# 0xPolygonZero/plonky2

Measured on NVIDIA H100. Metric: goldilocks_field_elements_per_s_ntt_lde_merkle, higher is better.
Workload: dtype u64

## Files before the change

include/plonky2_b200.h:

```cpp
#ifndef PLONKY2_B200_H
#define PLONKY2_B200_H
#include <stddef.h>
#include <stdint.h>

#ifdef __cplusplus
extern "C" {
#endif

#define GL_OK 0
#define GL_ERR_BAD_SHAPE 1
#define GL_ERR_OOM 2
#define GL_ERR_CUDA 3
#define GL_ERR_UNSUPPORTED 4
#define GL_ERR_BAD_ARG 5
#define GL_ERR_POW_FAILED 6
#define GL_ERR_DIV_ZERO 7

#define GL_MEM_HOST 0
#define GL_MEM_DEVICE 1

#define GL_SALT_SIZE 4

typedef struct gl_ctx gl_ctx;
typedef struct gl_commit gl_commit;
typedef struct gl_merkle gl_merkle;
typedef struct gl_fri gl_fri;

int gl_ctx_create(int device, void* stream, gl_ctx** out);
void gl_ctx_destroy(gl_ctx* ctx);
const char* gl_last_error(const gl_ctx* ctx);
int gl_ctx_synchronize(gl_ctx* ctx);
int gl_ctx_device_bytes(gl_ctx* ctx, uint64_t* in_use, uint64_t* high, int reset_high);
void* gl_ctx_stream(const gl_ctx* ctx);
uint64_t gl_ctx_launch_count(const gl_ctx* ctx);
int gl_ctx_set_ntt_group(gl_ctx* ctx, uint32_t columns);
#define GL_PHASE_INTT 0
#define GL_PHASE_LDE 1
#define GL_PHASE_LEAF_HASH 2
#define GL_PHASE_MERKLE_LEVELS 3
#define GL_NUM_PHASES 4
int gl_ctx_set_profiling(gl_ctx* ctx, int on);
int gl_ctx_phase_ms(gl_ctx* ctx, int phase, double* ms, uint64_t* count);
int gl_ctx_reset_phases(gl_ctx* ctx);

int gl_ntt(gl_ctx* ctx, uint64_t* data, uint32_t log_n, uint32_t batch, size_t stride, int inverse,
           uint32_t zero_factor_log, uint64_t coset_shift, int mem);

int gl_ntt_bcast(gl_ctx* ctx, const uint64_t* in, size_t in_stride, uint32_t log_n, uint32_t batch, int inverse,
                 uint64_t* const* outs, uint32_t n_outs, size_t out_stride);

int gl_bcast(gl_ctx* ctx, const uint64_t* src, size_t words, uint64_t* const* dests, uint32_t n_dests, uint32_t max_ctas);

int gl_commit_create(gl_ctx* ctx, const uint64_t* cols, size_t col_stride, uint32_t B, uint32_t log_n,
                     uint32_t rate_bits, uint32_t cap_height, const uint64_t* salt, int is_coeffs,
                     int mem, gl_commit** out);
int gl_commit_create_sharded(gl_ctx* ctx, const uint64_t* cols, size_t col_stride, uint32_t B, uint32_t log_n,
                             uint32_t rate_bits, uint32_t cap_height, const uint64_t* salt, int is_coeffs,
                             int mem, uint32_t shard_index, uint32_t num_shards, gl_commit** out);
#define GL_COLS_VALUES 0
#define GL_COLS_COEFFS 1
#define GL_COLS_COEFFS_CANONICAL 2
int gl_commit_begin(gl_ctx* ctx, uint32_t B, uint32_t log_n, uint32_t rate_bits, uint32_t cap_height, int blinding,
                    uint32_t shard_index, uint32_t num_shards, uint64_t* coeff_storage, gl_commit** out);
int gl_commit_add_columns(gl_commit* c, uint32_t first_col, uint32_t count, const uint64_t* cols, size_t col_stride,
                          int kind, int mem);
int gl_commit_finish(gl_commit* c, const uint64_t* salt, int mem);
int gl_commit_finish_keyed(gl_commit* c, const uint8_t key[32]);
int gl_commit_finish_prefixed(gl_commit* c, const uint64_t* prefix);
int gl_commit_begin_blocked(gl_ctx* ctx, uint32_t B, uint32_t log_n, uint32_t rate_bits, uint32_t cap_height,
                            uint32_t num_blocks, uint64_t* coeff_storage, gl_commit** out);
uint32_t gl_commit_lde_blocks(const gl_commit* c);
int gl_commit_shard(const gl_commit* c, uint32_t* shard_index, uint32_t* num_shards);
void gl_commit_destroy(gl_commit* c);
uint32_t gl_commit_num_polys(const gl_commit* c);
uint32_t gl_commit_leaf_width(const gl_commit* c);
uint32_t gl_commit_degree_log(const gl_commit* c);
uint32_t gl_commit_rate_bits(const gl_commit* c);
uint32_t gl_commit_cap_height(const gl_commit* c);
int gl_commit_cap(gl_commit* c, uint64_t* out, int mem);
int gl_commit_coeffs(gl_commit* c, uint64_t* out, int mem);
int gl_commit_leaves(gl_commit* c, size_t row_begin, size_t row_count, uint64_t* out, int mem);
int gl_commit_digests(gl_commit* c, uint64_t* out, int mem);
int gl_commit_get_lde_values(gl_commit* c, size_t index, size_t step, uint64_t* out);
int gl_commit_open(gl_commit* c, const uint64_t* leaf_indices, size_t count, uint64_t* out_leaves,
                   uint64_t* out_paths);
int gl_commit_eval_ext(gl_commit* c, const uint64_t point[2], uint64_t* out);
int gl_openings(gl_ctx* ctx, gl_commit* const* commits, const uint32_t* point_index, size_t n_evals,
                const uint64_t* points, size_t n_points, uint64_t* out, int mem);
int gl_openings_shard(gl_ctx* ctx, gl_commit* const* commits, const uint32_t* point_index, size_t n_evals,
                      const uint64_t* points, size_t n_points, uint32_t shard_index, uint32_t num_shards, uint64_t* out,
                      int mem);
const uint64_t* gl_commit_dev_lde(const gl_commit* c, size_t* col_stride);
const uint64_t* gl_commit_dev_coeffs(const gl_commit* c);
// ... 143 lines not shown
```

plonky2_b200/_native.py:

```python
import ctypes as C
import os

import numpy as np

HERE = os.path.dirname(os.path.abspath(__file__))
LIB_PATH = os.path.join(HERE, "libplonky2_b200.so")

GL_OK = 0
GL_ERR_BAD_SHAPE, GL_ERR_OOM, GL_ERR_CUDA, GL_ERR_UNSUPPORTED, GL_ERR_BAD_ARG, GL_ERR_POW_FAILED, GL_ERR_DIV_ZERO = 1, 2, 3, 4, 5, 6, 7
MEM_HOST, MEM_DEVICE = 0, 1
COLS_VALUES, COLS_COEFFS, COLS_COEFFS_CANONICAL = 0, 1, 2

u64p = C.POINTER(C.c_uint64)
u32p = C.POINTER(C.c_uint32)
vp = C.c_void_p

EXPORTS = [
    "gl_ctx_create", "gl_ctx_destroy", "gl_last_error", "gl_ctx_synchronize", "gl_ctx_launch_count",
    "gl_ctx_set_ntt_group", "gl_ctx_set_profiling", "gl_ctx_phase_ms", "gl_ctx_reset_phases", "gl_ctx_stream", "gl_ntt",
    "gl_ntt_bcast", "gl_bcast", "gl_commit_create", "gl_commit_create_sharded", "gl_commit_begin", "gl_commit_add_columns",
    "gl_commit_finish", "gl_commit_shard", "gl_commit_destroy", "gl_commit_num_polys",
    "gl_commit_leaf_width", "gl_commit_degree_log", "gl_commit_rate_bits", "gl_commit_cap_height",
    "gl_commit_cap", "gl_commit_coeffs", "gl_commit_leaves", "gl_commit_digests", "gl_commit_get_lde_values",
    "gl_commit_open", "gl_commit_eval_ext", "gl_openings", "gl_openings_shard", "gl_stark_quotient", "gl_stark_quotient_aux", "gl_stark_quotient_shard", "gl_stark_quotient_from_shards", "gl_stark_lookup_helpers", "gl_stark_ctl_helpers", "gl_plonk_quotient", "gl_plonk_quotient_shard", "gl_lookup_polys", "gl_sigma_polys", "gl_commit_dev_lde", "gl_commit_dev_coeffs", "gl_partial_products_and_zs", "gl_poseidon_permute_host",
    "gl_poseidon_permute_many", "gl_poseidon_hash_many", "gl_poseidon_hash_no_pad_many", "gl_poseidon_two_to_one_many", "gl_merkle_build", "gl_merkle_destroy",
    "gl_merkle_cap", "gl_merkle_digests", "gl_merkle_open", "gl_fri_begin", "gl_fri_begin_values", "gl_fri_values_local", "gl_fri_begin_from_coeffs",
    "gl_fri_destroy", "gl_fri_coeffs", "gl_fri_commit_round", "gl_fri_commit_round_sharded", "gl_fri_mix", "gl_fri_fold", "gl_fri_final_poly",
    "gl_fri_open", "gl_fri_num_rounds", "gl_fri_pow", "gl_commit_finish_keyed", "gl_random_field_elements",
    "gl_commit_finish_prefixed", "gl_commit_dev_cap", "gl_commit_begin_blocked", "gl_commit_lde_blocks",
    "gl_ctx_device_bytes",
]


class FriBatch(C.Structure):
    _fields_ = [("point", C.c_uint64 * 2), ("num_polys", C.c_size_t), ("oracle_index", u32p),
                ("poly_index", u32p)]


class ShapeError(ValueError):
    """Mirrors the reference's shape panics (fft.rs:171-177, merkle_tree.rs:195-200, oracle.rs:128)."""


class NativeError(RuntimeError):
    pass


_lib = None


def lib():
    global _lib
    if _lib is not None:
        return _lib
    if not os.path.exists(LIB_PATH):
        raise NativeError(
            "libplonky2_b200.so is not built (run `python -c 'import __graft_entry__ as g; g.build()'`); "
            "plonky2_b200 has no CPU fallback")
    L = C.CDLL(LIB_PATH)
    L.gl_ctx_create.argtypes = [C.c_int, vp, C.POINTER(vp)]
    L.gl_ctx_destroy.argtypes = [vp]
    L.gl_ctx_destroy.restype = None
    L.gl_last_error.argtypes = [vp]
    L.gl_last_error.restype = C.c_char_p
    L.gl_ctx_synchronize.argtypes = [vp]
    L.gl_ctx_device_bytes.argtypes = [vp, u64p, u64p, C.c_int]
    L.gl_ctx_launch_count.argtypes = [vp]
    L.gl_ctx_launch_count.restype = C.c_uint64
    L.gl_ctx_set_ntt_group.argtypes = [vp, C.c_uint32]
    L.gl_ntt.argtypes = [vp, vp, C.c_uint32, C.c_uint32, C.c_size_t, C.c_int, C.c_uint32, C.c_uint64, C.c_int]
    L.gl_ctx_stream.argtypes = [vp]
    L.gl_ctx_stream.restype = vp
    L.gl_ntt_bcast.argtypes = [vp, vp, C.c_size_t, C.c_uint32, C.c_uint32, C.c_int, C.POINTER(vp), C.c_uint32, C.c_size_t]
    L.gl_bcast.argtypes = [vp, vp, C.c_size_t, C.POINTER(vp), C.c_uint32, C.c_uint32]
    L.gl_commit_begin.argtypes = [vp, C.c_uint32, C.c_uint32, C.c_uint32, C.c_uint32, C.c_int, C.c_uint32, C.c_uint32,
                                  vp, C.POINTER(vp)]
    L.gl_commit_begin_blocked.argtypes = [vp, C.c_uint32, C.c_uint32, C.c_uint32, C.c_uint32, C.c_uint32, vp,
                                          C.POINTER(vp)]
    L.gl_commit_add_columns.argtypes = [vp, C.c_uint32, C.c_uint32, vp, C.c_size_t, C.c_int, C.c_int]
    L.gl_commit_finish.argtypes = [vp, vp, C.c_int]
    L.gl_commit_finish_keyed.argtypes = [vp, C.c_char_p]
    L.gl_commit_finish_prefixed.argtypes = [vp, vp]
    L.gl_random_field_elements.argtypes = [vp, C.c_char_p, C.c_uint32, C.c_uint64, C.c_size_t, vp, C.c_int]
    L.gl_commit_create.argtypes = [vp, vp, C.c_size_t, C.c_uint32, C.c_uint32, C.c_uint32, C.c_uint32, vp,
                                   C.c_int, C.c_int, C.POINTER(vp)]
    L.gl_commit_create_sharded.argtypes = [vp, vp, C.c_size_t, C.c_uint32, C.c_uint32, C.c_uint32, C.c_uint32, vp,
                                           C.c_int, C.c_int, C.c_uint32, C.c_uint32, C.POINTER(vp)]
    L.gl_commit_shard.argtypes = [vp, u32p, u32p]
    L.gl_ctx_set_profiling.argtypes = [vp, C.c_int]
    L.gl_ctx_phase_ms.argtypes = [vp, C.c_int, C.POINTER(C.c_double), C.POINTER(C.c_uint64)]
    L.gl_ctx_reset_phases.argtypes = [vp]
    L.gl_commit_destroy.argtypes = [vp]
    L.gl_commit_destroy.restype = None
    for n in ("gl_commit_num_polys", "gl_commit_leaf_width", "gl_commit_degree_log", "gl_commit_rate_bits",
              "gl_commit_cap_height", "gl_commit_lde_blocks"):
        getattr(L, n).argtypes = [vp]
        getattr(L, n).restype = C.c_uint32
    L.gl_commit_cap.argtypes = [vp, vp, C.c_int]
    L.gl_commit_coeffs.argtypes = [vp, vp, C.c_int]
    L.gl_commit_leaves.argtypes = [vp, C.c_size_t, C.c_size_t, vp, C.c_int]
    L.gl_commit_digests.argtypes = [vp, vp, C.c_int]
    L.gl_commit_get_lde_values.argtypes = [vp, C.c_size_t, C.c_size_t, vp]
    L.gl_commit_open.argtypes = [vp, vp, C.c_size_t, vp, vp]
    L.gl_commit_eval_ext.argtypes = [vp, vp, vp]
    L.gl_openings.argtypes = [vp, C.POINTER(vp), u32p, C.c_size_t, vp, C.c_size_t, vp, C.c_int]
    L.gl_openings_shard.argtypes = [vp, C.POINTER(vp), u32p, C.c_size_t, vp, C.c_size_t, C.c_uint32, C.c_uint32, vp,
                                    C.c_int]
    L.gl_stark_quotient.argtypes = [vp, vp, vp, C.c_uint32, vp, C.c_uint32, vp, C.c_uint32, C.c_uint32, vp]
    L.gl_stark_quotient_aux.argtypes = [vp, vp, vp, vp, C.c_uint32, vp, C.c_uint32, vp, C.c_uint32, C.c_uint32, vp]
    L.gl_stark_quotient_shard.argtypes = [vp, vp, vp, vp, C.c_uint32, vp, C.c_uint32, vp, C.c_uint32, C.c_uint32, vp]
    L.gl_stark_quotient_from_shards.argtypes = [vp, vp, C.c_uint32, C.c_uint32, C.c_uint32, C.c_uint32, vp]
    L.gl_stark_lookup_helpers.argtypes = [vp, vp, C.c_size_t, C.c_uint32, C.c_uint32, vp, u32p, C.c_uint32, vp,
                                          C.c_uint32, vp, C.c_uint32, C.c_uint32, vp]
    L.gl_stark_ctl_helpers.argtypes = [vp, vp, C.c_size_t, C.c_uint32, C.c_uint32, vp, u32p, C.c_uint32, vp, C.c_uint32,
                                       vp, C.c_uint32, C.c_uint32, u32p, vp]
    L.gl_plonk_quotient.argtypes = [vp, vp, C.c_uint32, vp, C.c_uint32, vp, C.c_uint32, vp, C.c_uint32, C.c_uint32,
                                    C.c_uint32, vp]
    L.gl_plonk_quotient_shard.argtypes = [vp, vp, C.c_uint32, vp, C.c_uint32, vp, C.c_uint32, vp, C.c_uint32,
                                          C.c_uint32, C.c_uint32, vp]
    L.gl_lookup_polys.argtypes = [vp, vp, C.c_uint32, C.c_uint32, C.c_uint32, vp, u32p, C.c_uint32, vp, C.c_int]
    L.gl_sigma_polys.argtypes = [vp, vp, C.c_size_t, C.c_int, C.c_uint32, C.c_uint32, C.c_uint32, C.c_uint64, vp, vp,
                                 C.c_int]
# ... 60 lines not shown

class Handle:
    destroyer = None
    h = None

    def close(self):
        if self.h:
            getattr(lib(), self.destroyer)(self.h)
            self.h = None

    def __del__(self):
        try:
            self.close()
        except Exception:
            pass


class Context(Handle):
    destroyer = "gl_ctx_destroy"
    _torch_stream = None

    def __init__(self, device=0, stream=None):
        h = vp()
        check(lib().gl_ctx_create(int(device), vp(stream) if stream else None, C.byref(h)))
        self.h = h
        self.device = device

    def synchronize(self):
        check(lib().gl_ctx_synchronize(self.h), self.h)

    def after_caller(self):
        import torch

        if self._torch_stream is None:
            self._torch_stream = torch.cuda.ExternalStream(self.stream, device=torch.device("cuda", self.device))
        self._torch_stream.wait_stream(torch.cuda.current_stream(self._torch_stream.device))

    @property
    def stream(self):
        return int(lib().gl_ctx_stream(self.h) or 0)

    def device_bytes(self, reset_high=False):
        in_use, high = C.c_uint64(), C.c_uint64()
        check(lib().gl_ctx_device_bytes(self.h, C.byref(in_use), C.byref(high), int(bool(reset_high))), self.h)
        return in_use.value, high.value

    @property
    def launch_count(self):
        return int(lib().gl_ctx_launch_count(self.h))

    def set_ntt_group(self, columns):
        check(lib().gl_ctx_set_ntt_group(self.h, int(columns)), self.h)

    PHASES = {"intt": 0, "lde": 1, "leaf_hash": 2, "merkle_levels": 3}

    def set_profiling(self, on):
        check(lib().gl_ctx_set_profiling(self.h, int(bool(on))), self.h)

    def reset_phases(self):
        check(lib().gl_ctx_reset_phases(self.h), self.h)

    def phase_ms(self):
        out = {}
        for name, pid in self.PHASES.items():
            ms, cnt = C.c_double(), C.c_uint64()
            check(lib().gl_ctx_phase_ms(self.h, pid, C.byref(ms), C.byref(cnt)), self.h)
            out[name] = (ms.value, cnt.value)
        return out


_default_ctx = {}


def default_context(device=0):
    if device not in _default_ctx:
        _default_ctx[device] = Context(device)
    return _default_ctx[device]
```

plonky2_b200/csrc/plonky2_b200.cu:

```cuda
#include <cooperative_groups.h>
#include <cub/device/device_radix_sort.cuh>
#include <cuda_runtime.h>

#include <cstdarg>
#include <cstdio>
#include <cstring>
#include <functional>
#include <initializer_list>
#include <map>
#include <memory>
#include <set>
#include <string>
#include <tuple>
#include <vector>

#include <sys/random.h>

#include <cerrno>

#include "../../include/plonky2_b200.h"
#include "gl_chacha.cuh"
#include "gl_field.cuh"
#include "gl_logup.cuh"
#include "gl_ctl.cuh"
#include "gl_ntt.cuh"
#include "gl_poseidon.cuh"
#include "gl_sigma.cuh"
#include "gl_vanishing.cuh"

using namespace gl;
typedef uint64_t u64;

static thread_local std::string g_last_error;

struct gl_ctx {
    int device = 0;
    cudaStream_t stream = nullptr;
    bool own_stream = false;
    u64 launches = 0;
    std::string err;
    std::map<std::tuple<int, u64, u64>, u64*> step_tabs;
    std::map<std::tuple<int, int, u64>, u64*> post_tabs;
    size_t table_bytes = 0;
    std::map<int, u64*> fold_tabs;
    cudaStream_t copy_stream = nullptr;
    std::set<const void*> smem_attr_done;
    u64* scratch = nullptr;
    size_t scratch_words = 0;
    u64* pinned = nullptr;
    size_t pinned_words = 0;
    u64* dstage = nullptr;
    size_t dstage_words = 0;
    uint32_t ntt_group = 0;
    int ntt_variant = 0;
    bool lde_per_coset = false;
    int sm_count = 0;
    int coop_ok = 0;
    int coop_blocks_per_sm = 0;
    bool prof_on = false;
    struct Pending {
        int phase;
        cudaEvent_t a, b;
    };
    std::vector<Pending> prof_pending;
    double prof_ms[GL_NUM_PHASES] = {0};
    u64 prof_count[GL_NUM_PHASES] = {0};
};

struct PhaseScope {
    gl_ctx* ctx;
    cudaEvent_t a = nullptr, b = nullptr;
    int phase;
    PhaseScope(gl_ctx* c, int ph) : ctx(c), phase(ph) {
        if (!ctx->prof_on) return;
        cudaEventCreate(&a);
        cudaEventCreate(&b);
        cudaEventRecord(a, ctx->stream);
    }
    ~PhaseScope() {
        if (!a) return;
        cudaEventRecord(b, ctx->stream);
        ctx->prof_pending.push_back({phase, a, b});
    }
};

static int set_err(gl_ctx* ctx, int code, const char* fmt, ...) {
    char buf[512];
    va_list ap;
    va_start(ap, fmt);
    vsnprintf(buf, sizeof(buf), fmt, ap);
    va_end(ap);
    g_last_error = buf;
    if (ctx) ctx->err = buf;
    return code;
}
#define CK(ctx, call)                                                                          \
    do {                                                                                       \
        cudaError_t e_ = (call);                                                               \
// ... 334 lines not shown
    }
}
__global__ void k_tree_open_prefixed(TreeView t, const u64* prefix, const u64* indices, u64* out_leaves,
                                     u64* out_paths) {
    const size_t idx = indices[blockIdx.x];
    const uint32_t num_layers = t.log_n - t.cap_height;
    const uint32_t lw = t.W + 4;
    for (uint32_t k = threadIdx.x; k < lw; k += blockDim.x)
        out_leaves[(size_t)blockIdx.x * lw + k] =
            canon(k < 4 ? prefix[4 * idx + k] : t.leaves[idx * t.ls + (size_t)(k - 4) * t.es]);
    const size_t L = (size_t)1 << num_layers;
    const size_t tree_index = idx >> num_layers;
    const u64* sub = t.digests + 4 * (tree_index * 2 * (L - 1));
    for (uint32_t k = threadIdx.x; k < num_layers * 4; k += blockDim.x) {
        const uint32_t i = k >> 2, w = k & 3;
        const size_t node = (idx & (L - 1)) >> i;
        out_paths[(size_t)blockIdx.x * num_layers * 4 + k] = sub[4 * digest_pos(node ^ 1, i) + w];
    }
}

struct Tree {
    u64* leaves = nullptr;
    u64* base = nullptr;
    bool own_leaves = false;
    u64* digests = nullptr;
    u64* cap = nullptr;
    u64* prefix = nullptr;
    size_t N = 0;
    size_t ls = 0, es = 1;
    uint32_t W = 0, log_n = 0, cap_height = 0;
    TreeView view() const { return TreeView{leaves, digests, cap, N, ls ? ls : (size_t)W, es, W, log_n, cap_height}; }
    size_t digest_words() const { return 8 * (N - ((size_t)1 << cap_height)); }
    size_t cap_words() const { return (size_t)4 << cap_height; }
};

static int log2_exact(size_t n, uint32_t* out) {
    if (n == 0 || (n & (n - 1))) return 1;
    uint32_t l = 0;
    while (((size_t)1 << l) < n) l++;
    *out = l;
    return 0;
}

static int tree_hash(gl_ctx* ctx, const Tree& t);
static int tree_build(gl_ctx* ctx, Tree& t) {
    if (log2_exact(t.N, &t.log_n)) return set_err(ctx, GL_ERR_BAD_SHAPE, "Not a power of two: %zu", t.N);
    if (t.cap_height > t.log_n)
        return set_err(ctx, GL_ERR_BAD_SHAPE, "cap_height=%u should be at most log2(leaves.len())=%u", t.cap_height,
                       t.log_n);
    TRY(dmalloc(ctx, &t.digests, t.digest_words()));
    TRY(dmalloc(ctx, &t.cap, t.cap_words()));
    return tree_hash(ctx, t);
}
static int tree_hash(gl_ctx* ctx, const Tree& t) {
    TreeView v = t.view();
    {
        PhaseScope ps(ctx, GL_PHASE_LEAF_HASH);
        const int cta = HASH_CTA;
        if (t.prefix)
            k_leaf_hash_prefixed<<<(unsigned)((t.N + cta - 1) / cta), cta, 0, ctx->stream>>>(v, t.prefix);
        else
            k_leaf_hash<<<(unsigned)((t.N + cta - 1) / cta), cta, 0, ctx->stream>>>(v);
        CKL(ctx);
    }
    PhaseScope ps2(ctx, GL_PHASE_MERKLE_LEVELS);
    const uint32_t sub_log = t.log_n - t.cap_height;
    const size_t coop_threads = ctx->coop_ok ? (size_t)ctx->coop_blocks_per_sm * ctx->sm_count * HASH_CTA : 0;
    for (uint32_t i = 1; i <= sub_log; i++) {
        size_t total = (size_t)1 << (t.log_n - i);
        if (coop_threads && total <= coop_threads && i < sub_log) {
            unsigned nb = (unsigned)((total + HASH_CTA - 1) / HASH_CTA);
            uint32_t i0 = i;
            void* args[] = {(void*)&v, (void*)&i0};
            CK(ctx, cudaLaunchCooperativeKernel((void*)k_merkle_upper, dim3(nb), dim3(HASH_CTA), args, 0, ctx->stream));
            ctx->launches++;
            break;
        }
        const int cta = HASH_CTA;
        k_merkle_level<<<(unsigned)((total + cta - 1) / cta), cta, 0, ctx->stream>>>(v, i);
        CKL(ctx);
    }
    return GL_OK;
}
static void tree_free(gl_ctx* ctx, Tree& t) {
    if (t.own_leaves) dfree(ctx, t.base ? t.base : t.leaves);
    dfree(ctx, t.digests);
    dfree(ctx, t.cap);
    dfree(ctx, t.prefix);
    t.leaves = t.digests = t.cap = t.prefix = nullptr;
}
static int tree_open(gl_ctx* ctx, const Tree& t, const u64* leaf_indices, size_t count, u64* out_leaves,
                     u64* out_paths) {
    if (count == 0) return GL_OK;
    for (size_t i = 0; i < count; i++)
        if (leaf_indices[i] >= t.N) return set_err(ctx, GL_ERR_BAD_ARG, "leaf index %llu out of range",
                                                   (unsigned long long)leaf_indices[i]);
    const uint32_t layers = t.log_n - t.cap_height;
    const size_t lw = count * (t.W + (t.prefix ? 4 : 0)), pw = count * layers * 4;
    TRY(ensure_dstage(ctx, count + lw + pw));
    TRY(ensure_pinned(ctx, count + lw + pw));
    CK(ctx, cudaStreamSynchronize(ctx->stream));
    memcpy(ctx->pinned, leaf_indices, count * 8);
    TRY(h2d(ctx, ctx->dstage, ctx->pinned, count));
    if (t.prefix)
        k_tree_open_prefixed<<<(unsigned)count, 128, 0, ctx->stream>>>(t.view(), t.prefix, ctx->dstage,
                                                                      ctx->dstage + count, ctx->dstage + count + lw);
    else
        k_tree_open<<<(unsigned)count, 128, 0, ctx->stream>>>(t.view(), ctx->dstage, ctx->dstage + count,
                                                             ctx->dstage + count + lw);
    CKL(ctx);
    TRY(d2h(ctx, ctx->pinned, ctx->dstage + count, lw + pw));
    memcpy(out_leaves, ctx->pinned, lw * 8);
    if (pw) memcpy(out_paths, ctx->pinned + lw, pw * 8);
    return GL_OK;
}

struct gl_commit {
    gl_ctx* ctx;
    uint32_t B, W, degree_log, rate_bits;
    uint32_t shard_index = 0, shard_log = 0;
    uint32_t lde_blocks = 0, block_log = 0;
    bool blinding;
    u64* coeffs = nullptr;
    bool own_coeffs = true;
    bool finished = false;
    Tree tree;
};

__global__ void k_salt(const u64* salt, size_t N, uint32_t log_N, size_t row0, size_t rows, u64* lde, size_t lde_stride,
                       uint32_t B) {
    size_t j = (size_t)blockIdx.x * blockDim.x + threadIdx.x;
    if (j >= rows) return;
    size_t i = (size_t)(__brevll(row0 + j) >> (64 - log_N));
    if (log_N == 0) i = 0;
    for (int s = 0; s < GL_SALT_SIZE; s++) lde[(size_t)(B + s) * lde_stride + j] = canon(salt[(size_t)s * N + i]);
}
__global__ void k_rows_from_columns(const u64* lde, size_t lde_stride, size_t row0, size_t rows, uint32_t W, u64* out) {
    __shared__ u64 tile[32][33];
    const size_t rb = (size_t)blockIdx.x * 32;
    const uint32_t kb = blockIdx.y * 32;
    for (int i = threadIdx.y; i < 32; i += blockDim.y) {
        const size_t r = rb + threadIdx.x;
        const uint32_t k = kb + i;
        if (r < rows && k < W) tile[i][threadIdx.x] = lde[(size_t)k * lde_stride + row0 + r];
    }
    __syncthreads();
    for (int i = threadIdx.y; i < 32; i += blockDim.y) {
        const size_t r = rb + i;
        const uint32_t k = kb + threadIdx.x;
        if (r < rows && k < W) out[r * W + k] = tile[threadIdx.x][i];
    }
}
__global__ void k_fold_coeffs(const u64* coeffs, size_t stride, size_t n, size_t M, u64 sM, u64* out) {
    size_t k0 = (size_t)blockIdx.x * blockDim.x + threadIdx.x;
    if (k0 >= M) return;
    const u64* col = coeffs + (size_t)blockIdx.y * stride;
    u64 acc = 0;
    for (size_t k1 = n / M; k1-- > 0;) acc = mul_add(acc, sM, col[k0 + M * k1]);
    out[(size_t)blockIdx.y * M + k0] = acc;
}
__global__ void k_canon(u64* data, size_t n) {
    size_t i = (size_t)blockIdx.x * blockDim.x + threadIdx.x;
    if (i < n) data[i] = canon(data[i]);
}
static int coset_lde_columns(gl_ctx* ctx, const u64* coeffs, uint32_t ncols, uint32_t log_n, uint32_t log_M, u64 shift,
                             u64* out, size_t out_stride) {
    const size_t n = (size_t)1 << log_n;
    if (log_M >= log_n) return lde_columns(ctx, coeffs, n, ncols, (int)log_n, (int)(log_M - log_n), shift, out, out_stride);
    const size_t M = (size_t)1 << log_M;
    DevBuf folded(ctx);
    TRY(folded.alloc((size_t)ncols * M));
    for (uint32_t b0 = 0; b0 < ncols; b0 += MAX_GRID_Y) {
        const uint32_t bc = (ncols - b0 < MAX_GRID_Y) ? ncols - b0 : MAX_GRID_Y;
        k_fold_coeffs<<<dim3((unsigned)((M + 127) / 128), bc), 128, 0, ctx->stream>>>(
            coeffs + (size_t)b0 * n, n, n, M, gl::pow(shift, M), folded.get() + (size_t)b0 * M);
        CKL(ctx);
    }
    return lde_columns(ctx, folded.get(), M, ncols, (int)log_M, 0, shift, out, out_stride);
}

static int commit_alloc(gl_ctx* ctx, gl_commit* c, uint32_t cap_height, u64* ext_coeffs) {
    const size_t n = (size_t)1 << c->degree_log, N = n << c->rate_bits;
    if (ext_coeffs) {
        c->coeffs = ext_coeffs;
        c->own_coeffs = false;
    } else {
        TRY(dmalloc(ctx, &c->coeffs, (size_t)c->B * n));
    }
    const uint32_t sl = c->shard_log;
    const size_t Nloc = N >> sl;
    Tree& t = c->tree;
    t.N = Nloc;
    t.W = c->W;
    t.log_n = c->degree_log + c->rate_bits - sl;
    t.cap_height = cap_height - sl;
    t.ls = 1;
    t.es = Nloc;
    if (c->lde_blocks) return GL_OK;
    t.own_leaves = true;
    TRY(dmalloc(ctx, &t.leaves, Nloc * (size_t)c->W));
    return GL_OK;
}
static int commit_extend(gl_ctx* ctx, const gl_commit* c, uint32_t g0, uint32_t gc, uint32_t g, uint32_t s, u64* out,
                         size_t out_stride) {
    PhaseScope ps(ctx, GL_PHASE_LDE);
    const u64 shift =
        mul(MULTIPLICATIVE_GROUP_GENERATOR, gl::pow(root_of_unity(c->degree_log + c->rate_bits), bitrev32(g, s)));
    return coset_lde_columns(ctx, c->coeffs + ((size_t)g0 << c->degree_log), gc, c->degree_log,
                             c->degree_log + c->rate_bits - s, shift, out, out_stride);
}
static int commit_chunk(gl_ctx* ctx, gl_commit* c, uint32_t g0, uint32_t gc, int kind) {
    const size_t n = (size_t)1 << c->degree_log;
    Tree& t = c->tree;
    u64* cg = c->coeffs + (size_t)g0 * n;
    if (kind == 0) {
        PhaseScope ps(ctx, GL_PHASE_INTT);
        TRY(ntt_natural(ctx, cg, n, cg, n, (int)c->degree_log, gc, true, 1));
    } else if (kind == 1) {
        size_t tot = (size_t)gc * n;
        k_canon<<<(unsigned)((tot + 255) / 256), 256, 0, ctx->stream>>>(cg, tot);
        CKL(ctx);
    }
    if (c->lde_blocks) return GL_OK;
    return commit_extend(ctx, c, g0, gc, c->shard_index, c->shard_log, t.leaves + (size_t)g0 * t.N, t.N);
}
static int commit_block(gl_ctx* ctx, const gl_commit* c, uint32_t g, DevBuf& scratch, Tree* out) {
    Tree t = c->tree;
    t.N >>= c->block_log;
    t.log_n -= c->block_log;
    t.cap_height -= c->block_log;
    t.es = t.N;
    if (t.cap) {
        t.digests += (size_t)g * t.digest_words();
        t.cap += (size_t)g * t.cap_words();
    }
    if (c->lde_blocks) {
        if (!scratch.get()) TRY(scratch.alloc((size_t)c->W * t.N));
        TRY(commit_extend(ctx, c, 0, c->B, g, c->block_log, scratch.get(), t.N));
        t.leaves = scratch.get();
    }
    *out = t;
    return GL_OK;
}
static int commit_finish(gl_ctx* ctx, gl_commit* c, const u64* salt, int mem, const ChaChaKey* key) {
    Tree& t = c->tree;
    const size_t Nloc = t.N;
    const uint32_t log_N = c->degree_log + c->rate_bits;
    HostReads reads(ctx);
    if (salt) {
        DevBuf dsalt(ctx);
        u64* sp;
        TRY(device_in(ctx, salt, (size_t)GL_SALT_SIZE << log_N, mem, dsalt, &sp));
        TRY(reads.mark(ctx->stream, mem));
        k_salt<<<(unsigned)((Nloc + 255) / 256), 256, 0, ctx->stream>>>(sp, (size_t)1 << log_N, log_N,
                                                                       (size_t)c->shard_index * Nloc, Nloc, t.leaves,
                                                                       Nloc, c->B);
        CKL(ctx);
    } else if (key) {
        const size_t items = salt_fill_items(log_N, Nloc);
        k_chacha_salt<<<dim3((unsigned)((items + 255) / 256), GL_SALT_SIZE), 256, 0, ctx->stream>>>(
            *key, log_N, (u64)c->shard_index * Nloc, Nloc, t.leaves + (size_t)c->B * Nloc, Nloc);
        CKL(ctx);
    }
    TRY(dmalloc(ctx, &t.digests, t.digest_words()));
    TRY(dmalloc(ctx, &t.cap, t.cap_words()));
    DevBuf scratch(ctx);
    for (uint32_t g = 0; g < (1u << c->block_log); g++) {
        Tree b;
        TRY(commit_block(ctx, c, g, scratch, &b));
        TRY(tree_hash(ctx, b));
    }
    TRY(reads.wait());
    c->finished = true;
    return GL_OK;
}
static int os_random_key(gl_ctx* ctx, uint8_t out[32]) {
    size_t got = 0;
    while (got < 32) {
        const ssize_t r = getrandom(out + got, 32 - got, 0);
        if (r < 0) {
            if (errno == EINTR) continue;
            return set_err(ctx, GL_ERR_UNSUPPORTED, "getrandom failed: %s", strerror(errno));
        }
        got += (size_t)r;
    }
    return GL_OK;
}

struct PolyRef {
    const u64* ptr;
    u64 a0, a1;
};
__global__ void k_fri_compose(const PolyRef* refs, uint32_t num, size_t n, u64* comp ) {
    size_t k = (size_t)blockIdx.x * blockDim.x + threadIdx.x;
    if (k >= n) return;
    Acc160 a0 = {0, 0, 0}, a1 = {0, 0, 0};
    for (uint32_t j = 0; j < num; j++) {
        const u64 c = refs[j].ptr[k];
        acc_mul(a0, c, refs[j].a0);
        acc_mul(a1, c, refs[j].a1);
    }
    comp[2 * k] = acc_reduce(a0);
    comp[2 * k + 1] = acc_reduce(a1);
}
__device__ __forceinline__ E2 e2_pow_tab(const u64* hi, const u64* lo, size_t m) {
    const size_t h = m >> 12, l = m & 4095;
    return e2_mul(E2{hi[2 * h], hi[2 * h + 1]}, E2{lo[2 * l], lo[2 * l + 1]});
}
__global__ void k_fill_e2_pows(E2 base, size_t count, u64* out) {
    size_t i = (size_t)blockIdx.x * blockDim.x + threadIdx.x;
    if (i >= count) return;
    E2 r = e2_pow(base, i);
    out[2 * i] = r.a;
    out[2 * i + 1] = r.b;
}
struct E2Pows4 {
    E2 base[4];
    size_t count[4];
    u64* out[4];
};
__global__ void k_fill_e2_pows4(E2Pows4 p) {
    size_t i = (size_t)blockIdx.x * blockDim.x + threadIdx.x;
#pragma unroll
// ... 729 lines not shown

extern "C" {

int gl_ctx_create(int device, void* stream, gl_ctx** out) {
    if (!out) return set_err(nullptr, GL_ERR_BAD_ARG, "out is NULL");
    *out = nullptr;
    int count = 0;
    cudaError_t e = cudaGetDeviceCount(&count);
    if (e != cudaSuccess || count == 0)
        return set_err(nullptr, GL_ERR_CUDA, "no CUDA device available (%s); this library has no CPU fallback",
                       cudaGetErrorString(e));
    if (device < 0 || device >= count) return set_err(nullptr, GL_ERR_BAD_ARG, "device %d out of range", device);
    gl_ctx* ctx = new gl_ctx();
    ctx->device = device;
    auto init = [&]() -> int {
        CK(ctx, cudaSetDevice(device));
        if (stream) {
            ctx->stream = (cudaStream_t)stream;
        } else {
            CK(ctx, cudaStreamCreateWithFlags(&ctx->stream, cudaStreamNonBlocking));
            ctx->own_stream = true;
        }
        CK(ctx, cudaDeviceGetAttribute(&ctx->sm_count, cudaDevAttrMultiProcessorCount, device));
        CK(ctx, cudaDeviceGetAttribute(&ctx->coop_ok, cudaDevAttrCooperativeLaunch, device));
        if (cudaOccupancyMaxActiveBlocksPerMultiprocessor(&ctx->coop_blocks_per_sm, k_merkle_upper, HASH_CTA, 0) !=
            cudaSuccess)
            ctx->coop_blocks_per_sm = 0;
        const PoseidonTables& t = host_poseidon_tables();
        CK(ctx, cudaMemcpyToSymbol(c_pos, &t, sizeof(PoseidonTables)));
        return GL_OK;
    };
    const int rc_init = init();
    if (rc_init != GL_OK) {
        if (ctx->own_stream) cudaStreamDestroy(ctx->stream);
        delete ctx;
        return rc_init;
    }
    cudaMemPool_t pool;
    if (cudaDeviceGetDefaultMemPool(&pool, device) == cudaSuccess) {
        unsigned long long thr = ~0ULL;
        cudaMemPoolSetAttribute(pool, cudaMemPoolAttrReleaseThreshold, &thr);
    }
    *out = ctx;
    return GL_OK;
}
void gl_ctx_destroy(gl_ctx* ctx) {
    if (!ctx) return;
    cudaSetDevice(ctx->device);
    cudaStreamSynchronize(ctx->stream);
    for (auto& kv : ctx->step_tabs) cudaFreeAsync(kv.second, ctx->stream);
    for (auto& kv : ctx->post_tabs) cudaFreeAsync(kv.second, ctx->stream);
    for (auto& kv : ctx->fold_tabs) cudaFreeAsync(kv.second, ctx->stream);
    if (ctx->copy_stream) cudaStreamDestroy(ctx->copy_stream);
    if (ctx->scratch) cudaFreeAsync(ctx->scratch, ctx->stream);
    if (ctx->dstage) cudaFreeAsync(ctx->dstage, ctx->stream);
    if (ctx->pinned) cudaFreeHost(ctx->pinned);
    cudaStreamSynchronize(ctx->stream);
    if (ctx->own_stream) cudaStreamDestroy(ctx->stream);
    delete ctx;
}
const char* gl_last_error(const gl_ctx* ctx) { return ctx ? ctx->err.c_str() : g_last_error.c_str(); }
int gl_ctx_synchronize(gl_ctx* ctx) {
    CK(ctx, cudaStreamSynchronize(ctx->stream));
    return GL_OK;
}
int gl_ctx_device_bytes(gl_ctx* ctx, uint64_t* in_use, uint64_t* high, int reset_high) {
    if (!ctx) return set_err(ctx, GL_ERR_BAD_ARG, "null context");
    CK(ctx, cudaSetDevice(ctx->device));
    CK(ctx, cudaStreamSynchronize(ctx->stream));
    cudaMemPool_t pool;
    CK(ctx, cudaDeviceGetDefaultMemPool(&pool, ctx->device));
    uint64_t v = 0;
    CK(ctx, cudaMemPoolGetAttribute(pool, cudaMemPoolAttrUsedMemCurrent, &v));
    if (in_use) *in_use = v;
    CK(ctx, cudaMemPoolGetAttribute(pool, cudaMemPoolAttrUsedMemHigh, &v));
    if (high) *high = v;
    if (reset_high) {
        uint64_t zero = 0;
        CK(ctx, cudaMemPoolSetAttribute(pool, cudaMemPoolAttrUsedMemHigh, &zero));
    }
    return GL_OK;
}
uint64_t gl_ctx_launch_count(const gl_ctx* ctx) { return ctx->launches; }
int gl_ctx_set_ntt_group(gl_ctx* ctx, uint32_t columns) {
    ctx->ntt_variant = (columns >> 31) & 1;
    ctx->lde_per_coset = (columns >> 30) & 1;
    ctx->ntt_group = columns & 0x3FFFFFFFu;
    return GL_OK;
}
int gl_ctx_set_profiling(gl_ctx* ctx, int on) {
    ctx->prof_on = on != 0;
    return GL_OK;
}
int gl_ctx_phase_ms(gl_ctx* ctx, int phase, double* ms, uint64_t* count) {
    if (phase < 0 || phase >= GL_NUM_PHASES) return set_err(ctx, GL_ERR_BAD_ARG, "bad phase");
    if (!ctx->prof_pending.empty()) {
        CK(ctx, cudaStreamSynchronize(ctx->stream));
        for (auto& p : ctx->prof_pending) {
            float t = 0;
            cudaEventElapsedTime(&t, p.a, p.b);
            ctx->prof_ms[p.phase] += t;
            ctx->prof_count[p.phase]++;
            cudaEventDestroy(p.a);
            cudaEventDestroy(p.b);
        }
        ctx->prof_pending.clear();
    }
    if (ms) *ms = ctx->prof_ms[phase];
    if (count) *count = ctx->prof_count[phase];
    return GL_OK;
}
int gl_ctx_reset_phases(gl_ctx* ctx) {
    TRY(gl_ctx_phase_ms(ctx, 0, nullptr, nullptr));
    for (int i = 0; i < GL_NUM_PHASES; i++) {
        ctx->prof_ms[i] = 0;
        ctx->prof_count[i] = 0;
    }
    return GL_OK;
}

int gl_ntt(gl_ctx* ctx, uint64_t* data, uint32_t log_n, uint32_t batch, size_t stride, int inverse,
           uint32_t zero_factor_log, uint64_t coset_shift, int mem) {
    (void)zero_factor_log;
    if (!ctx || !data) return set_err(ctx, GL_ERR_BAD_ARG, "null argument");
    CK(ctx, cudaSetDevice(ctx->device));
    if (log_n > 3 * NTT_MAX_LOG_PASS) return set_err(ctx, GL_ERR_UNSUPPORTED, "log_n %u > 30", log_n);
    const size_t n = (size_t)1 << log_n;
    if (batch > 1 && stride < n) return set_err(ctx, GL_ERR_BAD_SHAPE, "stride %zu < n %zu", stride, n);
    if (canon(coset_shift) == 0) return set_err(ctx, GL_ERR_BAD_ARG, "coset_shift must be non-zero");
    if (mem == GL_MEM_DEVICE) return ntt_natural(ctx, data, stride, data, stride, (int)log_n, batch, inverse != 0, coset_shift);
    DevBuf d(ctx);
    TRY(d.alloc((size_t)batch * n));
    const size_t pitch = (batch > 1 ? stride : n) * 8;
    if (cudaMemcpy2DAsync(d.get(), n * 8, data, pitch, n * 8, batch, cudaMemcpyHostToDevice, ctx->stream) != cudaSuccess)
        return set_err(ctx, GL_ERR_CUDA, "H2D: %s", cudaGetErrorString(cudaGetLastError()));
    TRY(ntt_natural(ctx, d.get(), n, d.get(), n, (int)log_n, batch, inverse != 0, coset_shift));
    cudaError_t e = cudaMemcpy2DAsync(data, pitch, d.get(), n * 8, n * 8, batch, cudaMemcpyDeviceToHost, ctx->stream);
    if (e != cudaSuccess) return set_err(ctx, GL_ERR_CUDA, "D2H: %s", cudaGetErrorString(e));
    if (cudaStreamSynchronize(ctx->stream) != cudaSuccess)
        return set_err(ctx, GL_ERR_CUDA, "sync failed: %s", cudaGetErrorString(cudaGetLastError()));
    return GL_OK;
// ... 79 lines not shown
                    uint32_t shard_index, uint32_t num_shards, uint64_t* coeff_storage, gl_commit** out) {
    if (!ctx || !out) return set_err(ctx, GL_ERR_BAD_ARG, "null argument");
    *out = nullptr;
    uint32_t shard_log = 0;
    TRY(commit_check_shape(ctx, B, log_n, rate_bits, cap_height, shard_index, num_shards, &shard_log));
    CK(ctx, cudaSetDevice(ctx->device));
    CommitPtr c = commit_new(ctx, B, log_n, rate_bits, blinding != 0, shard_index, shard_log);
    TRY(commit_alloc(ctx, c.get(), cap_height, coeff_storage));
    *out = c.release();
    return GL_OK;
}
int gl_commit_begin_blocked(gl_ctx* ctx, uint32_t B, uint32_t log_n, uint32_t rate_bits, uint32_t cap_height,
                            uint32_t num_blocks, uint64_t* coeff_storage, gl_commit** out) {
    if (!ctx || !out) return set_err(ctx, GL_ERR_BAD_ARG, "null argument");
    *out = nullptr;
    uint32_t shard_log = 0, block_log = 0;
    TRY(commit_check_shape(ctx, B, log_n, rate_bits, cap_height, 0, 1, &shard_log));
    if (log2_exact(num_blocks, &block_log) || block_log > cap_height)
        return set_err(ctx, GL_ERR_BAD_SHAPE,
                       "num_blocks=%u: a power of two of at most the cap size 2^%u (blocks own whole cap subtrees)",
                       num_blocks, cap_height);
    CK(ctx, cudaSetDevice(ctx->device));
    CommitPtr c = commit_new(ctx, B, log_n, rate_bits, false, 0, 0);
    c->lde_blocks = num_blocks;
    c->block_log = block_log;
    TRY(commit_alloc(ctx, c.get(), cap_height, coeff_storage));
    *out = c.release();
    return GL_OK;
}
#define NEED_HANDLE(c)                                                         \
    do {                                                                       \
        if (!(c)) return set_err(nullptr, GL_ERR_BAD_ARG, "null handle");       \
    } while (0)
#define NEED_FINISHED(c)                                                                                     \
    do {                                                                                                     \
        NEED_HANDLE(c);                                                                                      \
        if (!(c)->finished) return set_err((c)->ctx, GL_ERR_BAD_ARG, "gl_commit_finish has not been called"); \
    } while (0)
int gl_commit_add_columns(gl_commit* c, uint32_t first_col, uint32_t count, const uint64_t* cols, size_t col_stride,
                          int kind, int mem) {
    NEED_HANDLE(c);
    gl_ctx* ctx = c->ctx;
    if (c->finished) return set_err(ctx, GL_ERR_BAD_ARG, "commitment already finished");
    if (!cols || kind < 0 || kind > 2) return set_err(ctx, GL_ERR_BAD_ARG, "bad argument");
    if (count == 0) return GL_OK;
    if ((size_t)first_col + count > c->B) return set_err(ctx, GL_ERR_BAD_SHAPE, "columns %u..%u outside the batch of %u", first_col, first_col + count, c->B);
    const size_t n = (size_t)1 << c->degree_log;
    if (count > 1 && col_stride < n) return set_err(ctx, GL_ERR_BAD_SHAPE, "Polynomial degrees inconsistent (stride < n)");
    CK(ctx, cudaSetDevice(ctx->device));
    u64* dst = c->coeffs + (size_t)first_col * n;
    const uint32_t CH = 32, CH0 = 8;
    if (mem != GL_MEM_HOST || count <= CH) {
        HostReads reads(ctx);
        if (!(mem == GL_MEM_DEVICE && cols == dst && (col_stride == n || count == 1)))
            CK(ctx, cudaMemcpy2DAsync(dst, n * 8, cols, col_stride * 8, n * 8, count,
                                      mem == GL_MEM_HOST ? cudaMemcpyHostToDevice : cudaMemcpyDeviceToDevice,
                                      ctx->stream));
        TRY(reads.mark(ctx->stream, mem));
        TRY(commit_chunk(ctx, c, first_col, count, kind));
        return reads.wait();
    }
    struct EventList {
        std::vector<cudaEvent_t> v;
        ~EventList() {
            for (auto e : v) cudaEventDestroy(e);
        }
    } evs;
    std::vector<std::pair<uint32_t, uint32_t>> chunks;
    for (uint32_t k0 = 0; k0 < count;) {
        const uint32_t want = k0 == 0 ? CH0 : CH, kc = (count - k0 < want) ? count - k0 : want;
        chunks.emplace_back(k0, kc);
        k0 += kc;
    }
    if (!ctx->copy_stream) CK(ctx, cudaStreamCreateWithFlags(&ctx->copy_stream, cudaStreamNonBlocking));
    cudaEvent_t ready;
    CK(ctx, cudaEventCreateWithFlags(&ready, cudaEventDisableTiming));
    CK(ctx, cudaEventRecord(ready, ctx->stream));
    CK(ctx, cudaStreamWaitEvent(ctx->copy_stream, ready, 0));
    cudaEventDestroy(ready);
    for (auto& ch : chunks) {
        const uint32_t k0 = ch.first, kc = ch.second;
        if (col_stride == n) {
            CK(ctx, cudaMemcpyAsync(dst + (size_t)k0 * n, cols + (size_t)k0 * n, (size_t)kc * n * 8,
                                    cudaMemcpyHostToDevice, ctx->copy_stream));
        } else {
            CK(ctx, cudaMemcpy2DAsync(dst + (size_t)k0 * n, n * 8, cols + (size_t)k0 * col_stride, col_stride * 8, n * 8,
                                      kc, cudaMemcpyHostToDevice, ctx->copy_stream));
        }
        cudaEvent_t e;
        CK(ctx, cudaEventCreateWithFlags(&e, cudaEventDisableTiming));
        CK(ctx, cudaEventRecord(e, ctx->copy_stream));
        evs.v.push_back(e);
    }
    HostReads reads(ctx);
    TRY(reads.mark(ctx->copy_stream, mem));
    for (size_t k = 0; k < chunks.size(); k++) {
        CK(ctx, cudaStreamWaitEvent(ctx->stream, evs.v[k], 0));
        TRY(commit_chunk(ctx, c, first_col + chunks[k].first, chunks[k].second, kind));
    }
    return reads.wait();
}
int gl_commit_finish(gl_commit* c, const uint64_t* salt, int mem) {
    NEED_HANDLE(c);
    gl_ctx* ctx = c->ctx;
    if (c->finished) return set_err(ctx, GL_ERR_BAD_ARG, "commitment already finished");
    if (c->blinding != (salt != nullptr)) return set_err(ctx, GL_ERR_BAD_ARG, "salt must be given exactly when blinding was requested");
    CK(ctx, cudaSetDevice(ctx->device));
    return commit_finish(ctx, c, salt, mem, nullptr);
}
int gl_commit_finish_prefixed(gl_commit* c, const uint64_t* prefix) {
    NEED_HANDLE(c);
    gl_ctx* ctx = c->ctx;
// ... 1462 lines not shown
```

Before: 8.491 billion.

## Overlap coset LDE with leaf hashing on a side stream; skip device copy before INTT

Adds an optional pipelined commit path that splits the LDE into power-of-two coset blocks. Each block is computed on a separate priority stream while the previous block's leaves are hashed, synchronised with events, and the Merkle levels are then built once. It also lets the inverse NTT read device value columns directly instead of first copying them into the coefficient buffer, which removes one device-to-device copy. The pipeline is controlled by a new commit_blocks setting that defaults to 1, so it stays off unless configured; when on, it adds stream and event overhead and smaller per-block kernels.

```diff
diff --git a/include/plonky2_b200.h b/include/plonky2_b200.h
--- a/include/plonky2_b200.h
+++ b/include/plonky2_b200.h
@@ -34,11 +34,13 @@
 void* gl_ctx_stream(const gl_ctx* ctx);
 uint64_t gl_ctx_launch_count(const gl_ctx* ctx);
 int gl_ctx_set_ntt_group(gl_ctx* ctx, uint32_t columns);
+int gl_ctx_set_commit_blocks(gl_ctx* ctx, uint32_t blocks);
 #define GL_PHASE_INTT 0
 #define GL_PHASE_LDE 1
 #define GL_PHASE_LEAF_HASH 2
 #define GL_PHASE_MERKLE_LEVELS 3
-#define GL_NUM_PHASES 4
+#define GL_PHASE_LDE_UNDER_HASH 4
+#define GL_NUM_PHASES 5
 int gl_ctx_set_profiling(gl_ctx* ctx, int on);
 int gl_ctx_phase_ms(gl_ctx* ctx, int phase, double* ms, uint64_t* count);
 int gl_ctx_reset_phases(gl_ctx* ctx);
diff --git a/plonky2_b200/_native.py b/plonky2_b200/_native.py
--- a/plonky2_b200/_native.py
+++ b/plonky2_b200/_native.py
@@ -28,7 +28,7 @@
     "gl_fri_destroy", "gl_fri_coeffs", "gl_fri_commit_round", "gl_fri_commit_round_sharded", "gl_fri_mix", "gl_fri_fold", "gl_fri_final_poly",
     "gl_fri_open", "gl_fri_num_rounds", "gl_fri_pow", "gl_commit_finish_keyed", "gl_random_field_elements",
     "gl_commit_finish_prefixed", "gl_commit_dev_cap", "gl_commit_begin_blocked", "gl_commit_lde_blocks",
-    "gl_ctx_device_bytes",
+    "gl_ctx_device_bytes", "gl_ctx_set_commit_blocks",
 ]
 
 
@@ -67,6 +67,7 @@
     L.gl_ctx_launch_count.argtypes = [vp]
     L.gl_ctx_launch_count.restype = C.c_uint64
     L.gl_ctx_set_ntt_group.argtypes = [vp, C.c_uint32]
+    L.gl_ctx_set_commit_blocks.argtypes = [vp, C.c_uint32]
     L.gl_ntt.argtypes = [vp, vp, C.c_uint32, C.c_uint32, C.c_size_t, C.c_int, C.c_uint32, C.c_uint64, C.c_int]
     L.gl_ctx_stream.argtypes = [vp]
     L.gl_ctx_stream.restype = vp
@@ -233,6 +234,9 @@
     def set_ntt_group(self, columns):
         check(lib().gl_ctx_set_ntt_group(self.h, int(columns)), self.h)
 
+    def set_commit_blocks(self, blocks):
+        check(lib().gl_ctx_set_commit_blocks(self.h, int(blocks)), self.h)
+
     PHASES = {"intt": 0, "lde": 1, "leaf_hash": 2, "merkle_levels": 3}
 
     def set_profiling(self, on):
diff --git a/plonky2_b200/csrc/plonky2_b200.cu b/plonky2_b200/csrc/plonky2_b200.cu
--- a/plonky2_b200/csrc/plonky2_b200.cu
+++ b/plonky2_b200/csrc/plonky2_b200.cu
@@ -44,6 +44,9 @@
     size_t table_bytes = 0;
     std::map<int, u64*> fold_tabs;
     cudaStream_t copy_stream = nullptr;
+    uint32_t commit_blocks = 1;
+    cudaStream_t lde_stream = nullptr;
+    int lde_stream_priority = 0;
     std::set<const void*> smem_attr_done;
     u64* scratch = nullptr;
     size_t scratch_words = 0;
@@ -484,17 +487,25 @@
     TRY(dmalloc(ctx, &t.cap, t.cap_words()));
     return tree_hash(ctx, t);
 }
+static int leaf_hash(gl_ctx* ctx, const Tree& t) {
+    const int cta = HASH_CTA;
+    if (t.prefix)
+        k_leaf_hash_prefixed<<<(unsigned)((t.N + cta - 1) / cta), cta, 0, ctx->stream>>>(t.view(), t.prefix);
+    else
+        k_leaf_hash<<<(unsigned)((t.N + cta - 1) / cta), cta, 0, ctx->stream>>>(t.view());
+    CKL(ctx);
+    return GL_OK;
+}
+static int merkle_levels(gl_ctx* ctx, const Tree& t);
 static int tree_hash(gl_ctx* ctx, const Tree& t) {
-    TreeView v = t.view();
     {
         PhaseScope ps(ctx, GL_PHASE_LEAF_HASH);
-        const int cta = HASH_CTA;
-        if (t.prefix)
-            k_leaf_hash_prefixed<<<(unsigned)((t.N + cta - 1) / cta), cta, 0, ctx->stream>>>(v, t.prefix);
-        else
-            k_leaf_hash<<<(unsigned)((t.N + cta - 1) / cta), cta, 0, ctx->stream>>>(v);
-        CKL(ctx);
-    }
+        TRY(leaf_hash(ctx, t));
+    }
+    return merkle_levels(ctx, t);
+}
+static int merkle_levels(gl_ctx* ctx, const Tree& t) {
+    TreeView v = t.view();
     PhaseScope ps2(ctx, GL_PHASE_MERKLE_LEVELS);
     const uint32_t sub_log = t.log_n - t.cap_height;
     const size_t coop_threads = ctx->coop_ok ? (size_t)ctx->coop_blocks_per_sm * ctx->sm_count * HASH_CTA : 0;
@@ -513,6 +524,21 @@
         CKL(ctx);
     }
     return GL_OK;
+}
+static Tree block_view(const Tree& t, uint32_t s, uint32_t g) {
+    Tree b = t;
+    b.own_leaves = false;
+    b.N >>= s;
+    b.log_n -= s;
+    b.cap_height -= s;
+    const size_t row0 = (size_t)g * b.N;
+    if (b.leaves) b.leaves += row0 * (b.ls ? b.ls : b.W);
+    if (b.prefix) b.prefix += 4 * row0;
+    if (b.cap) {
+        b.digests += (size_t)g * b.digest_words();
+        b.cap += (size_t)g * b.cap_words();
+    }
+    return b;
 }
 static void tree_free(gl_ctx* ctx, Tree& t) {
     if (t.own_leaves) dfree(ctx, t.base ? t.base : t.leaves);
@@ -552,6 +578,7 @@
     uint32_t B, W, degree_log, rate_bits;
     uint32_t shard_index = 0, shard_log = 0;
     uint32_t lde_blocks = 0, block_log = 0;
+    uint32_t pipe_log = 0;
     bool blinding;
     u64* coeffs = nullptr;
     bool own_coeffs = true;
@@ -611,6 +638,13 @@
     return lde_columns(ctx, folded.get(), M, ncols, (int)log_M, 0, shift, out, out_stride);
 }
 
+static uint32_t pipeline_log(uint32_t blocks, uint32_t rate_bits, uint32_t cap_height) {
+    uint32_t want = 0;
+    while ((2u << want) <= blocks) want++;
+    if (want > rate_bits) want = rate_bits;
+    if (want > cap_height) want = cap_height;
+    return want;
+}
 static int commit_alloc(gl_ctx* ctx, gl_commit* c, uint32_t cap_height, u64* ext_coeffs) {
     const size_t n = (size_t)1 << c->degree_log, N = n << c->rate_bits;
     if (ext_coeffs) {
@@ -629,50 +663,122 @@
     t.ls = 1;
     t.es = Nloc;
     if (c->lde_blocks) return GL_OK;
+    c->pipe_log = pipeline_log(ctx->commit_blocks, c->rate_bits > sl ? c->rate_bits - sl : 0, t.cap_height);
     t.own_leaves = true;
     TRY(dmalloc(ctx, &t.leaves, Nloc * (size_t)c->W));
     return GL_OK;
 }
 static int commit_extend(gl_ctx* ctx, const gl_commit* c, uint32_t g0, uint32_t gc, uint32_t g, uint32_t s, u64* out,
                          size_t out_stride) {
-    PhaseScope ps(ctx, GL_PHASE_LDE);
     const u64 shift =
         mul(MULTIPLICATIVE_GROUP_GENERATOR, gl::pow(root_of_unity(c->degree_log + c->rate_bits), bitrev32(g, s)));
     return coset_lde_columns(ctx, c->coeffs + ((size_t)g0 << c->degree_log), gc, c->degree_log,
                              c->degree_log + c->rate_bits - s, shift, out, out_stride);
 }
-static int commit_chunk(gl_ctx* ctx, gl_commit* c, uint32_t g0, uint32_t gc, int kind) {
+static int commit_chunk(gl_ctx* ctx, gl_commit* c, uint32_t g0, uint32_t gc, int kind, const u64* src = nullptr,
+                        size_t src_stride = 0) {
     const size_t n = (size_t)1 << c->degree_log;
     Tree& t = c->tree;
     u64* cg = c->coeffs + (size_t)g0 * n;
     if (kind == 0) {
         PhaseScope ps(ctx, GL_PHASE_INTT);
-        TRY(ntt_natural(ctx, cg, n, cg, n, (int)c->degree_log, gc, true, 1));
+        TRY(ntt_natural(ctx, src ? src : cg, src ? src_stride : n, cg, n, (int)c->degree_log, gc, true, 1));
     } else if (kind == 1) {
         size_t tot = (size_t)gc * n;
         k_canon<<<(unsigned)((tot + 255) / 256), 256, 0, ctx->stream>>>(cg, tot);
         CKL(ctx);
     }
-    if (c->lde_blocks) return GL_OK;
+    if (c->lde_blocks || c->pipe_log) return GL_OK;
+    PhaseScope ps(ctx, GL_PHASE_LDE);
     return commit_extend(ctx, c, g0, gc, c->shard_index, c->shard_log, t.leaves + (size_t)g0 * t.N, t.N);
 }
 static int commit_block(gl_ctx* ctx, const gl_commit* c, uint32_t g, DevBuf& scratch, Tree* out) {
-    Tree t = c->tree;
-    t.N >>= c->block_log;
-    t.log_n -= c->block_log;
-    t.cap_height -= c->block_log;
-    t.es = t.N;
-    if (t.cap) {
-        t.digests += (size_t)g * t.digest_words();
-        t.cap += (size_t)g * t.cap_words();
-    }
+    Tree t = block_view(c->tree, c->block_log, g);
     if (c->lde_blocks) {
         if (!scratch.get()) TRY(scratch.alloc((size_t)c->W * t.N));
+        PhaseScope ps(ctx, GL_PHASE_LDE);
         TRY(commit_extend(ctx, c, 0, c->B, g, c->block_log, scratch.get(), t.N));
         t.leaves = scratch.get();
+        t.es = t.N;
     }
     *out = t;
     return GL_OK;
+}
+class OnStream {
+  public:
+    OnStream(gl_ctx* ctx, cudaStream_t s) : ctx_(ctx), saved_(ctx->stream) { ctx->stream = s; }
+    OnStream(const OnStream&) = delete;
+    OnStream& operator=(const OnStream&) = delete;
+    ~OnStream() { ctx_->stream = saved_; }
+
+  private:
+    gl_ctx* ctx_;
+    cudaStream_t saved_;
+};
+class SideEvents {
+  public:
+    SideEvents(gl_ctx* ctx, cudaStream_t side) : ctx_(ctx), side_(side) {}
+    SideEvents(const SideEvents&) = delete;
+    SideEvents& operator=(const SideEvents&) = delete;
+    ~SideEvents() {
+        cudaEvent_t e;
+        if (cudaEventCreateWithFlags(&e, cudaEventDisableTiming) == cudaSuccess) {
+            cudaEventRecord(e, side_);
+            cudaStreamWaitEvent(ctx_->stream, e, 0);
+            cudaEventDestroy(e);
+        } else {
+            cudaStreamSynchronize(side_);
+        }
+        for (auto e2 : v_) cudaEventDestroy(e2);
+    }
+    int record(cudaStream_t s, cudaEvent_t* out) {
+        CK(ctx_, cudaEventCreateWithFlags(out, cudaEventDisableTiming));
+        v_.push_back(*out);
+        CK(ctx_, cudaEventRecord(*out, s));
+        return GL_OK;
+    }
+
+  private:
+    gl_ctx* ctx_;
+    cudaStream_t side_;
+    std::vector<cudaEvent_t> v_;
+};
+static int commit_lde_under_hash(gl_ctx* ctx, const gl_commit* c) {
+    const Tree& t = c->tree;
+    const uint32_t s = c->pipe_log, G = 1u << s;
+    if (!ctx->lde_stream)
+        CK(ctx, cudaStreamCreateWithPriority(&ctx->lde_stream, cudaStreamNonBlocking, ctx->lde_stream_priority));
+    cudaStream_t hash_stream = ctx->stream, side = ctx->lde_stream;
+    SideEvents ev(ctx, side);
+    std::vector<cudaEvent_t> lde_done(G), hash_done(G);
+    cudaEvent_t ready;
+    TRY(ev.record(hash_stream, &ready));
+    CK(ctx, cudaStreamWaitEvent(side, ready, 0));
+    auto extend = [&](uint32_t g) -> int {
+        OnStream on(ctx, side);
+        const Tree b = block_view(t, s, g);
+        TRY(commit_extend(ctx, c, 0, c->B, (c->shard_index << s) + g, c->shard_log + s, b.leaves, t.N));
+        return ev.record(side, &lde_done[g]);
+    };
+    {
+        OnStream on(ctx, side);
+        PhaseScope ps(ctx, GL_PHASE_LDE);
+        TRY(extend(0));
+    }
+    CK(ctx, cudaStreamWaitEvent(hash_stream, lde_done[0], 0));
+    {
+        PhaseScope ps(ctx, GL_PHASE_LDE_UNDER_HASH);
+        for (uint32_t g = 0; g < G; g++) {
+            if (g + 1 < G) {
+                if (g >= 1) CK(ctx, cudaStreamWaitEvent(side, hash_done[g - 1], 0));
+                TRY(extend(g + 1));
+            }
+            if (g >= 1) CK(ctx, cudaStreamWaitEvent(hash_stream, lde_done[g], 0));
+            TRY(leaf_hash(ctx, block_view(t, s, g)));
+            TRY(ev.record(hash_stream, &hash_done[g]));
+        }
+    }
+    return merkle_levels(ctx, t);
 }
 static int commit_finish(gl_ctx* ctx, gl_commit* c, const u64* salt, int mem, const ChaChaKey* key) {
     Tree& t = c->tree;
@@ -696,11 +802,15 @@
     }
     TRY(dmalloc(ctx, &t.digests, t.digest_words()));
     TRY(dmalloc(ctx, &t.cap, t.cap_words()));
-    DevBuf scratch(ctx);
-    for (uint32_t g = 0; g < (1u << c->block_log); g++) {
-        Tree b;
-        TRY(commit_block(ctx, c, g, scratch, &b));
-        TRY(tree_hash(ctx, b));
+    if (c->pipe_log) {
+        TRY(commit_lde_under_hash(ctx, c));
+    } else {
+        DevBuf scratch(ctx);
+        for (uint32_t g = 0; g < (1u << c->block_log); g++) {
+            Tree b;
+            TRY(commit_block(ctx, c, g, scratch, &b));
+            TRY(tree_hash(ctx, b));
+        }
     }
     TRY(reads.wait());
     c->finished = true;
@@ -1536,6 +1646,7 @@
     for (auto& kv : ctx->post_tabs) cudaFreeAsync(kv.second, ctx->stream);
     for (auto& kv : ctx->fold_tabs) cudaFreeAsync(kv.second, ctx->stream);
     if (ctx->copy_stream) cudaStreamDestroy(ctx->copy_stream);
+    if (ctx->lde_stream) cudaStreamDestroy(ctx->lde_stream);
     if (ctx->scratch) cudaFreeAsync(ctx->scratch, ctx->stream);
     if (ctx->dstage) cudaFreeAsync(ctx->dstage, ctx->stream);
     if (ctx->pinned) cudaFreeHost(ctx->pinned);
@@ -1571,6 +1682,50 @@
     ctx->lde_per_coset = (columns >> 30) & 1;
     ctx->ntt_group = columns & 0x3FFFFFFFu;
     return GL_OK;
+}
+int gl_ctx_set_commit_blocks(gl_ctx* ctx, uint32_t blocks) {
+    if (!ctx) return set_err(ctx, GL_ERR_BAD_ARG, "null context");
+    if (blocks == 0 || (blocks & (blocks - 1)))
+        return set_err(ctx, GL_ERR_BAD_ARG, "commit blocks %u: not a power of two", blocks);
+    ctx->commit_blocks = blocks;
+    return GL_OK;
+}
+int gl_debug_lde_stream_priority(gl_ctx* ctx, int priority) {
+    if (!ctx) return set_err(ctx, GL_ERR_BAD_ARG, "null context");
+    CK(ctx, cudaSetDevice(ctx->device));
+    if (ctx->lde_stream) {
+        CK(ctx, cudaStreamSynchronize(ctx->lde_stream));
+        CK(ctx, cudaStreamDestroy(ctx->lde_stream));
+        ctx->lde_stream = nullptr;
+    }
+    ctx->lde_stream_priority = priority;
+    return GL_OK;
+}
+uint32_t gl_debug_pipeline_log(uint32_t blocks, uint32_t rate_bits, uint32_t cap_height) {
+    return pipeline_log(blocks, rate_bits, cap_height);
+}
+void gl_debug_block_view(size_t N, uint32_t W, uint32_t cap_height, uint32_t s, uint32_t g, size_t out[7]) {
+    Tree t;
+    uint32_t log_n = 0;
+    log2_exact(N, &log_n);
+    u64* const base = reinterpret_cast<u64*>((uintptr_t)1 << 40);
+    t.leaves = base;
+    t.digests = base + ((size_t)1 << 36);
+    t.cap = base + ((size_t)2 << 36);
+    t.N = N;
+    t.ls = 1;
+    t.es = N;
+    t.W = W;
+    t.log_n = log_n;
+    t.cap_height = cap_height;
+    const Tree b = block_view(t, s, g);
+    out[0] = (size_t)(b.leaves - t.leaves);
+    out[1] = b.es;
+    out[2] = b.N;
+    out[3] = b.log_n;
+    out[4] = b.cap_height;
+    out[5] = (size_t)(b.digests - t.digests);
+    out[6] = (size_t)(b.cap - t.cap);
 }
 int gl_ctx_set_profiling(gl_ctx* ctx, int on) {
     ctx->prof_on = on != 0;
@@ -1756,12 +1911,17 @@
     const uint32_t CH = 32, CH0 = 8;
     if (mem != GL_MEM_HOST || count <= CH) {
         HostReads reads(ctx);
-        if (!(mem == GL_MEM_DEVICE && cols == dst && (col_stride == n || count == 1)))
+        const size_t stride = count > 1 ? col_stride : n;
+        const bool in_place = mem == GL_MEM_DEVICE && cols == dst && (col_stride == n || count == 1);
+        const uintptr_t s0 = (uintptr_t)cols, s1 = (uintptr_t)(cols + (size_t)(count - 1) * stride + n);
+        const uintptr_t d0 = (uintptr_t)dst, d1 = (uintptr_t)(dst + (size_t)count * n);
+        const bool from_cols = mem == GL_MEM_DEVICE && kind == GL_COLS_VALUES && !in_place && (s1 <= d0 || d1 <= s0);
+        if (!in_place && !from_cols)
             CK(ctx, cudaMemcpy2DAsync(dst, n * 8, cols, col_stride * 8, n * 8, count,
                                       mem == GL_MEM_HOST ? cudaMemcpyHostToDevice : cudaMemcpyDeviceToDevice,
                                       ctx->stream));
         TRY(reads.mark(ctx->stream, mem));
-        TRY(commit_chunk(ctx, c, first_col, count, kind));
+        TRY(commit_chunk(ctx, c, first_col, count, kind, from_cols ? cols : nullptr, stride));
         return reads.wait();
     }
     struct EventList {
```

Measured after the change: 8.576 billion, median of 6. +1.0%, better.
